# cmhungsteve/TA3N

Measured on NVIDIA H100. Metric: video-clips/sec fwd+bwd (B=256,T=5,D=2048), higher is better.
Workload: dtype tf32x3

## Files before the change

ta3n_b200/csrc/gemm_wgmma.cuh:

```cuda
#pragma once

#include <cuda.h>
#include <stdlib.h>

#include <algorithm>
#include <cmath>
#include <functional>
#include <map>
#include <tuple>

#include "seg_gemm.cuh"

namespace ta3n {

constexpr int TC_BM = 128, TC_BN = 128, TC_BK = 32;
constexpr int TC_THREADS = 384;
constexpr int TC_CONSUMER_WARPS = 8;
constexpr int TC_B_WARPS = 3;
constexpr int TC_B_THREADS = 32 * TC_B_WARPS;
constexpr int TC_PRODUCER_REGS = 40, TC_CONSUMER_REGS = 232;
static_assert(128 * TC_PRODUCER_REGS + 256 * TC_CONSUMER_REGS <= TC_THREADS * 168,
              "setmaxnreg budget exceeds the registers of one CTA");
constexpr int TC_XPOSE_PRODUCER_REGS = 64, TC_XPOSE_CONSUMER_REGS = 216;
static_assert(128 * TC_XPOSE_PRODUCER_REGS + 256 * TC_XPOSE_CONSUMER_REGS <= TC_THREADS * 168,
// ... 45 lines not shown
  } while (!done);
}
__device__ __forceinline__ void mbar_arrive(uint64_t* bar) {
  asm volatile("mbarrier.arrive.shared::cta.b64 _, [%0];" ::"r"(smem_u32(bar)) : "memory");
}
__device__ __forceinline__ void fence_barrier_init() { asm volatile("fence.mbarrier_init.release.cluster;" ::: "memory"); }
__device__ __forceinline__ void fence_proxy_async() { asm volatile("fence.proxy.async.shared::cta;" ::: "memory"); }

__device__ __forceinline__ void tma_load_2d(void* smem_dst, const CUtensorMap* map, uint64_t* bar, int c0, int c1) {
  asm volatile(
      "cp.async.bulk.tensor.2d.shared::cluster.global.mbarrier::complete_tx::bytes [%0], [%1, {%3, %4}], [%2];"
      ::"r"(smem_u32(smem_dst)), "l"(map), "r"(smem_u32(bar)), "r"(c0), "r"(c1)
      : "memory");
}
__device__ __forceinline__ void tma_load_3d(void* smem_dst, const CUtensorMap* map, uint64_t* bar, int c0, int c1,
                                            int c2) {
  asm volatile(
      "cp.async.bulk.tensor.3d.shared::cluster.global.mbarrier::complete_tx::bytes [%0], [%1, {%3, %4, %5}], [%2];"
      ::"r"(smem_u32(smem_dst)), "l"(map), "r"(smem_u32(bar)), "r"(c0), "r"(c1), "r"(c2)
      : "memory");
}
__device__ __forceinline__ void tma_prefetch_2d(const CUtensorMap* map, int c0, int c1) {
  asm volatile("cp.async.bulk.prefetch.tensor.2d.L2.global.tile [%0, {%1, %2}];" ::"l"(map), "r"(c0), "r"(c1) : "memory");
}
__device__ __forceinline__ void tma_prefetch_3d(const CUtensorMap* map, int c0, int c1, int c2) {
  asm volatile("cp.async.bulk.prefetch.tensor.3d.L2.global.tile [%0, {%1, %2, %3}];" ::"l"(map), "r"(c0), "r"(c1), "r"(c2)
               : "memory");
}
__device__ __forceinline__ void tma_prefetch_desc(const CUtensorMap* map) {
  asm volatile("prefetch.tensormap [%0];" ::"l"(map) : "memory");
}

__device__ __forceinline__ void sts4(uint32_t saddr, const float4 v) {
  asm volatile("st.shared.v4.f32 [%0], {%1, %2, %3, %4};" ::"r"(saddr), "f"(v.x), "f"(v.y), "f"(v.z), "f"(v.w) : "memory");
}
__device__ __forceinline__ float4 lds4(uint32_t saddr) {
  float4 v;
  asm volatile("ld.shared.v4.f32 {%0, %1, %2, %3}, [%4];" : "=f"(v.x), "=f"(v.y), "=f"(v.z), "=f"(v.w) : "r"(saddr) : "memory");
  return v;
}
__device__ __forceinline__ void wgmma_fence() { asm volatile("wgmma.fence.sync.aligned;" ::: "memory"); }
__device__ __forceinline__ void wgmma_commit() { asm volatile("wgmma.commit_group.sync.aligned;" ::: "memory"); }
template <int N>
__device__ __forceinline__ void wgmma_wait() {
  asm volatile("wgmma.wait_group.sync.aligned %0;" ::"n"(N) : "memory");
}

__device__ __forceinline__ uint64_t wgmma_desc(uint32_t tile_base, int kstep) {
  const uint32_t a = tile_base + (uint32_t)kstep * 32u;
  return (uint64_t)((a >> 4) & 0x3FFF) | ((uint64_t)1 << 16) | ((uint64_t)(1024 >> 4) << 32) | ((uint64_t)1 << 62);
}

__device__ __forceinline__ void wgmma_tf32(float (&d)[64], uint64_t adesc, uint64_t bdesc) {
  asm volatile(
      "{\n\t.reg .pred p;\n\t"
      "setp.ne.b32 p, %66, 0;\n\t"
      "wgmma.mma_async.sync.aligned.m64n128k8.f32.tf32.tf32 "
      "{%0, %1, %2, %3, %4, %5, %6, %7, %8, %9, %10, %11, %12, %13, %14, %15, %16, %17, %18, %19, %20, %21, %22, %23, %24, %25, %26, %27, %28, %29, %30, %31, %32, %33, %34, %35, %36, %37, %38, %39, %40, %41, %42, %43, %44, %45, %46, %47, %48, %49, %50, %51, %52, %53, %54, %55, %56, %57, %58, %59, %60, %61, %62, %63}, %64, %65, p, 1, 1;\n\t}"
      : "+f"(d[0]), "+f"(d[1]), "+f"(d[2]), "+f"(d[3]), "+f"(d[4]), "+f"(d[5]), "+f"(d[6]), "+f"(d[7]), "+f"(d[8]), "+f"(d[9]), "+f"(d[10]), "+f"(d[11]), "+f"(d[12]), "+f"(d[13]), "+f"(d[14]), "+f"(d[15]), "+f"(d[16]), "+f"(d[17]), "+f"(d[18]), "+f"(d[19]), "+f"(d[20]), "+f"(d[21]), "+f"(d[22]), "+f"(d[23]), "+f"(d[24]), "+f"(d[25]), "+f"(d[26]), "+f"(d[27]), "+f"(d[28]), "+f"(d[29]), "+f"(d[30]), "+f"(d[31]), "+f"(d[32]), "+f"(d[33]), "+f"(d[34]), "+f"(d[35]), "+f"(d[36]), "+f"(d[37]), "+f"(d[38]), "+f"(d[39]), "+f"(d[40]), "+f"(d[41]), "+f"(d[42]), "+f"(d[43]), "+f"(d[44]), "+f"(d[45]), "+f"(d[46]), "+f"(d[47]), "+f"(d[48]), "+f"(d[49]), "+f"(d[50]), "+f"(d[51]), "+f"(d[52]), "+f"(d[53]), "+f"(d[54]), "+f"(d[55]), "+f"(d[56]), "+f"(d[57]), "+f"(d[58]), "+f"(d[59]), "+f"(d[60]), "+f"(d[61]), "+f"(d[62]), "+f"(d[63])
      : "l"(adesc), "l"(bdesc), "r"(1)
      : "memory");
}
__device__ __forceinline__ void wgmma_tf32_rs(float (&d)[64], const uint32_t a0, const uint32_t a1, const uint32_t a2,
                                              const uint32_t a3, uint64_t bdesc) {
  asm volatile(
      "{\n\t.reg .pred p;\n\t"
      "setp.ne.b32 p, %69, 0;\n\t"
      "wgmma.mma_async.sync.aligned.m64n128k8.f32.tf32.tf32 "
      "{%0, %1, %2, %3, %4, %5, %6, %7, %8, %9, %10, %11, %12, %13, %14, %15, %16, %17, %18, %19, %20, %21, %22, %23, %24, %25, %26, %27, %28, %29, %30, %31, %32, %33, %34, %35, %36, %37, %38, %39, %40, %41, %42, %43, %44, %45, %46, %47, %48, %49, %50, %51, %52, %53, %54, %55, %56, %57, %58, %59, %60, %61, %62, %63}, {%64, %65, %66, %67}, %68, p, 1, 1;\n\t}"
      : "+f"(d[0]), "+f"(d[1]), "+f"(d[2]), "+f"(d[3]), "+f"(d[4]), "+f"(d[5]), "+f"(d[6]), "+f"(d[7]), "+f"(d[8]), "+f"(d[9]), "+f"(d[10]), "+f"(d[11]), "+f"(d[12]), "+f"(d[13]), "+f"(d[14]), "+f"(d[15]), "+f"(d[16]), "+f"(d[17]), "+f"(d[18]), "+f"(d[19]), "+f"(d[20]), "+f"(d[21]), "+f"(d[22]), "+f"(d[23]), "+f"(d[24]), "+f"(d[25]), "+f"(d[26]), "+f"(d[27]), "+f"(d[28]), "+f"(d[29]), "+f"(d[30]), "+f"(d[31]), "+f"(d[32]), "+f"(d[33]), "+f"(d[34]), "+f"(d[35]), "+f"(d[36]), "+f"(d[37]), "+f"(d[38]), "+f"(d[39]), "+f"(d[40]), "+f"(d[41]), "+f"(d[42]), "+f"(d[43]), "+f"(d[44]), "+f"(d[45]), "+f"(d[46]), "+f"(d[47]), "+f"(d[48]), "+f"(d[49]), "+f"(d[50]), "+f"(d[51]), "+f"(d[52]), "+f"(d[53]), "+f"(d[54]), "+f"(d[55]), "+f"(d[56]), "+f"(d[57]), "+f"(d[58]), "+f"(d[59]), "+f"(d[60]), "+f"(d[61]), "+f"(d[62]), "+f"(d[63])
      : "r"(a0), "r"(a1), "r"(a2), "r"(a3), "l"(bdesc), "r"(1)
      : "memory");
}
__device__ __forceinline__ void reg_fence(uint32_t& r) { asm volatile("" : "+r"(r)::"memory"); }
__device__ __forceinline__ float lds1(uint32_t saddr) {
  float v;
  asm volatile("ld.shared.f32 %0, [%1];" : "=f"(v) : "r"(saddr) : "memory");
  return v;
}
template <int N>
__device__ __forceinline__ void setmaxnreg_dec() { asm volatile("setmaxnreg.dec.sync.aligned.u32 %0;" ::"n"(N)); }
template <int N>
__device__ __forceinline__ void setmaxnreg_inc() { asm volatile("setmaxnreg.inc.sync.aligned.u32 %0;" ::"n"(N)); }

__device__ __forceinline__ uint32_t kmaj_chunk(int m, int kq) { return (uint32_t)(m * 128 + ((kq ^ (m & 7)) << 4)); }
__device__ __forceinline__ uint32_t mnmaj_chunk(int k, int mq) {
  return (uint32_t)((mq >> 3) * 4096 + k * 128 + (((mq & 7) ^ (k & 7)) << 4));
}
__device__ __forceinline__ float tf32_hi(float a) { return __uint_as_float(__float_as_uint(a) & 0xFFFFE000u); }
__device__ __forceinline__ float f4_at(const float4& v, int i) { return i == 0 ? v.x : i == 1 ? v.y : i == 2 ? v.z : v.w; }

__device__ __forceinline__ void tc_prep_blk(const int t, int* mq, int* kq) {
  *mq = (t & 3) | (((t >> 3) & 7) << 2);
  *kq = ((t >> 2) & 1) | ((((t >> 1) ^ (t >> 7)) & 1) << 1) | (((t >> 6) & 1) << 2);
}
__device__ __forceinline__ void tc_prep_load(const uint32_t base, const int t, float4 (&r)[4]) {
  int mq, kq;
  tc_prep_blk(t, &mq, &kq);
  const uint32_t p = base + (uint32_t)((mq >> 3) * 4096 + 512 * kq + (((mq & 7) ^ (4 * (kq & 1))) << 4));
#pragma unroll
  for (int i = 0; i < 4; ++i) r[i] = lds4((p ^ (i << 4)) + 128u * i);
}
__device__ __forceinline__ void tc_prep_store(const uint32_t base, const int t, const float4 (&r)[4]) {
  int mq, kq;
  tc_prep_blk(t, &mq, &kq);
  const uint32_t p = base + (uint32_t)(512 * mq + ((kq ^ (4 * (mq & 1))) << 4));
#pragma unroll
  for (int i = 0; i < 4; ++i)
    sts4((p ^ (i << 4)) + 128u * i, make_float4(f4_at(r[0], i), f4_at(r[1], i), f4_at(r[2], i), f4_at(r[3], i)));
}
static_assert(2 * TC_B_THREADS < 256 && 256 <= 3 * TC_B_THREADS, "tc_transpose_b moves two or three blocks per thread");
template <bool TWO_IN_FLIGHT>
__device__ __forceinline__ void tc_transpose_b(const uint32_t b_mn, const uint32_t b_k, const int t) {
  if (!TWO_IN_FLIGHT) {
#pragma unroll 1
    for (int blk = t; blk < 256; blk += TC_B_THREADS) {
      float4 r[4];
      tc_prep_load(b_mn, blk, r);
      tc_prep_store(b_k, blk, r);
    }
    return;
  }
  const bool third = t + 2 * TC_B_THREADS < 256;
  float4 r[4], q[4];
  tc_prep_load(b_mn, t, r);
  tc_prep_load(b_mn, t + TC_B_THREADS, q);
  tc_prep_store(b_k, t, r);
  if (third) tc_prep_load(b_mn, t + 2 * TC_B_THREADS, r);
  tc_prep_store(b_k, t + TC_B_THREADS, q);
  if (third) tc_prep_store(b_k, t + 2 * TC_B_THREADS, r);
}

template <bool A_KMAJ>
__device__ __forceinline__ uint32_t tc_a_thread_off(const int m, const int tq) {
  return A_KMAJ ? kmaj_chunk(m, 0) + 4u * tq : mnmaj_chunk(tq, m >> 2) + 4u * (m & 3);
}

template <bool A_KMAJ>
__device__ __forceinline__ void tc_load_a(const uint32_t a_base, const uint32_t off0, const uint32_t off1,
                                          uint32_t (&a)[16]) {
  const uint32_t p0 = a_base + off0, p1 = a_base + off1;
#pragma unroll
  for (int ks = 0; ks < TC_BK / 8; ++ks)
#pragma unroll
    for (int j = 0; j < 4; ++j) {
      const uint32_t row = j & 1, half = j >> 1;
      const uint32_t addr = A_KMAJ ? (p0 ^ ((2u * ks + half) << 4)) + 1024u * row
                                   : ((row ? p1 : p0) ^ (half << 6)) + 512u * half + 1024u * ks;
      a[4 * ks + j] = __float_as_uint(lds1(addr));
    }
}

#ifdef TA3N_TC_TIMELINE
constexpr int kTlCtas = 132, kTlSlabs = 64, kTlEvents = 9;
enum : int {
  TL_TMA_ISSUE,
  TL_FULL,
  TL_XPOSE_START,
  TL_XPOSE_END,
  TL_CONS_START,
  TL_READY,
  TL_RELEASED,
  TL_RETIRED,
  TL_FENCE,
};
__device__ unsigned long long g_tc_tl[kTlCtas][kTlSlabs][kTlEvents];
__device__ unsigned long long g_tc_tl_clk[kTlCtas][4];
__device__ __forceinline__ unsigned long long tl_globaltimer() {
  unsigned long long t;
  asm volatile("mov.u64 %0, %%globaltimer;" : "=l"(t));
  return t;
}
__device__ __forceinline__ void tl_stamp(const uint32_t slab, const int ev) {
  if (blockIdx.x < kTlCtas && slab < (uint32_t)kTlSlabs) g_tc_tl[blockIdx.x][slab][ev] = clock64();
}
__device__ __forceinline__ void tl_clock(const int at_end) {
  if (blockIdx.x < kTlCtas) {
    g_tc_tl_clk[blockIdx.x][2 * at_end] = tl_globaltimer();
    g_tc_tl_clk[blockIdx.x][2 * at_end + 1] = clock64();
  }
}
#define TA3N_TL(cond, slab, ev) \
  do {                          \
    if (cond) tl_stamp((uint32_t)(slab), (ev)); \
  } while (0)
#else
#define TA3N_TL(cond, slab, ev) ((void)0)
#endif

struct TcShared {
  uint64_t full_bar[kTcMaxStages];
  uint64_t empty_bar[kTcMaxStages];
};

template <int STAGES>
__device__ __forceinline__ void tc_pipe_init(TcShared* sh, const int readers = TC_CONSUMER_WARPS) {
  for (int s = 0; s < STAGES; ++s) {
    mbar_init(&sh->full_bar[s], 1);
    mbar_init(&sh->empty_bar[s], readers);
  }
  fence_barrier_init();
}

template <int STAGES, int STAGE_BYTES = TC_STAGE_BYTES>
__device__ __forceinline__ void tc_produce(const TileCtx& ctx, const CUtensorMap* __restrict__ maps, const bool a_kmaj,
                                           const bool b_kmaj, const int pad_flags, const int m0, const int n0,
                                           const int c_begin, const int n_iter, uint8_t* smem, TcShared* sh,
                                           const uint32_t slabs) {
  const Group& g = ctx.g;
  int seg = 0, k0 = 0;
  {
    int skip = c_begin;
    while (seg < g.seg_count) {
      const int nch = (ctx.seg[seg].len + TC_BK - 1) / TC_BK;
      if (skip < nch) {
        k0 = skip * TC_BK;
        break;
      }
      skip -= nch;
      ++seg;
    }
  }
  for (int it = 0; it < n_iter; ++it) {
    const uint32_t gl = slabs + (uint32_t)it;
    const int stage = (int)(gl % STAGES);
    const uint32_t phase = (gl / STAGES) & 1u;
    mbar_wait(&sh->empty_bar[stage], phase ^ 1u);
    TA3N_TL(true, gl, TL_TMA_ISSUE);
    mbar_expect_tx(&sh->full_bar[stage], TC_STAGE_BYTES);
    uint8_t* sA = smem + stage * STAGE_BYTES;
    uint8_t* sB = sA + TC_A_BYTES;
    const CUtensorMap* ma = &maps[ctx.seg[seg].amap];
    const CUtensorMap* mb = &maps[ctx.seg[seg].bmap];
    if (a_kmaj) {
      tma_load_2d(sA, ma, &sh->full_bar[stage], k0, m0);
    } else if (pad_flags & 1) {
      tma_load_3d(sA, ma, &sh->full_bar[stage], 0, k0, m0 >> 5);
    } else {
#pragma unroll
      for (int q = 0; q < TC_BM / 32; ++q) tma_load_2d(sA + q * 4096, ma, &sh->full_bar[stage], m0 + 32 * q, k0);
    }
    if (b_kmaj) {
      tma_load_2d(sB, mb, &sh->full_bar[stage], k0, n0);
    } else if (pad_flags & 2) {
      tma_load_3d(sB, mb, &sh->full_bar[stage], 0, k0, n0 >> 5);
    } else {
#pragma unroll
      for (int q = 0; q < TC_BN / 32; ++q) tma_load_2d(sB + q * 4096, mb, &sh->full_bar[stage], n0 + 32 * q, k0);
    }
    k0 += TC_BK;
    if (k0 >= ctx.seg[seg].len) {
      ++seg;
      k0 = 0;
    }
  }
}

__device__ __forceinline__ void tc_chunk_range(const TileCtx& ctx, int split, int* c_begin, int* n_iter) {
  const Group& g = ctx.g;
  int total_chunks = 0;
  for (int s = 0; s < g.seg_count; ++s) total_chunks += (ctx.seg[s].len + TC_BK - 1) / TC_BK;
  const int cps = (total_chunks + g.ksplit - 1) / g.ksplit;
  *c_begin = split * cps;
  *n_iter = max(0, min(total_chunks, *c_begin + cps) - *c_begin);
}

__device__ __forceinline__ void tc_decode(const TileCtx& ctx, const int tile, int* split, int* m0, int* n0) {
  const Group& g = ctx.g;
  int local = tile - g.tile_begin;
  const int per_split = g.tiles_m * g.tiles_n;
  *split = local / per_split;
  local -= *split * per_split;
  *m0 = (local / g.tiles_n) * TC_BM;
  *n0 = (local % g.tiles_n) * TC_BN;
}

__device__ __forceinline__ void frag_st2(float* p, const float x0, const float x1, const bool vec, const bool two) {
  if (vec) {
    *reinterpret_cast<float2*>(p) = make_float2(x0, x1);
  } else {
    p[0] = x0;
    if (two) p[1] = x1;
  }
}

template <int F>
__device__ __forceinline__ void frag_epilogue(const Group& g, const int m0, const int n0, const float (&v)[64]) {
  constexpr bool kFwd = F >= 0 && (F & ~(EPI_BIAS | EPI_RELU | EPI_DROP_RNG)) == 0;
  const int M = g.M, N = g.N, ldc = g.ldc;
  float* const C = g.C;
  const bool vec = (N % 2) == 0 && (ldc % 2) == 0 && (reinterpret_cast<uintptr_t>(C) & 7u) == 0;
  const float alpha = kFwd ? (g.alpha_dev ? g.alpha * __ldg(g.alpha_dev) : g.alpha) : 0.f;
  const float* const bias = g.bias;
  const uint64_t seed = g.seed, roff = g.rng_offset;
  const uint64_t step = (kFwd && (F & EPI_DROP_RNG) && g.step_dev) ? *g.step_dev : 0ull;
  const float dscale = g.drop_scale, dp = g.drop_p;
  const uint32_t thr = rng_threshold(dp);
  float b0[16], b1[16];
#pragma unroll
  for (int j = 0; j < 16; ++j) {
    const int n = n0 + 8 * j;
    b0[j] = kFwd && (F & EPI_BIAS) && n < N ? bias[n] : 0.f;
    b1[j] = kFwd && (F & EPI_BIAS) && n + 1 < N ? bias[n + 1] : 0.f;
  }
#pragma unroll
  for (int h = 0; h < 2; ++h) {
    const int m = m0 + 8 * h;
    if (m >= M) continue;
#pragma unroll
    for (int j = 0; j < 16; ++j) {
      const int n = n0 + 8 * j;
      if (n >= N) continue;
      const bool two = n + 1 < N;
      float x0 = v[4 * j + 2 * h], x1 = v[4 * j + 2 * h + 1];
      if (kFwd) {
        x0 *= alpha;
        x1 *= alpha;
        if (F & EPI_BIAS) {
          x0 += b0[j];
          x1 += b1[j];
        }
        if (F & EPI_RELU) {
          x0 = fmaxf(x0, 0.0f);
          x1 = fmaxf(x1, 0.0f);
        }
        if (F & EPI_DROP_RNG) {
          const uint64_t e = roff + (uint64_t)m * (uint64_t)N + (uint64_t)n;
          bool k0, k1;
          if ((e & 1ull) == 0) {
            const uint64_t hsh = rng_hash4(seed, step, e >> 2);
            k0 = rng_keep_bits(hsh, (int)(e & 3ull), thr);
            k1 = rng_keep_bits(hsh, (int)(e & 3ull) + 1, thr);
          } else {
            k0 = rng_keep(seed, step, e, dp);
            k1 = rng_keep(seed, step, e + 1, dp);
          }
          const float f0 = k0 ? dscale : 0.0f, f1 = k1 ? dscale : 0.0f;
          x0 = f0 != 0.0f ? x0 * f0 : 0.0f;
          x1 = f1 != 0.0f ? x1 * f1 : 0.0f;
        }
      } else {
        x0 = epilogue_t<F>(g, m, n, x0);
        if (two) x1 = epilogue_t<F>(g, m, n + 1, x1);
      }
      frag_st2(C + (size_t)m * ldc + n, x0, x1, vec, two);
    }
  }
}

__device__ __forceinline__ void frag_finish(const Group& g, const int split, const int tm0, const int tn0,
                                            const float (&v)[64]) {
  const int warp = threadIdx.x >> 5, lane = threadIdx.x & 31;
  const int m0 = tm0 + (warp >> 2) * 64 + (warp & 3) * 16 + (lane >> 2), n0 = tn0 + 2 * (lane & 3);
  if (g.ksplit > 1) {
    const int M = g.M, N = g.N;
    float* const part = g.partial + (size_t)split * M * N;
    const bool vec = (N % 2) == 0;
#pragma unroll
    for (int h = 0; h < 2; ++h)
#pragma unroll
      for (int j = 0; j < 16; ++j) {
        const int m = m0 + 8 * h, n = n0 + 8 * j;
        if (m < M && n < N) frag_st2(part + (size_t)m * N + n, v[4 * j + 2 * h], v[4 * j + 2 * h + 1], vec, n + 1 < N);
      }
    return;
  }
  TA3N_EPI_DISPATCH(g.flags, { frag_epilogue<EPI_F>(g, m0, n0, v); })
}


template <bool A_KMAJ, bool B_KMAJ>
__device__ __forceinline__ void tc_consume_slab(const uint32_t it, uint8_t* smem, TcShared* sh, uint64_t* kready_bar,
                                                uint64_t* kempty_bar, const uint32_t off0, const uint32_t off1,
                                                uint32_t (&a)[16], float (&d)[64], int& prev) {
  constexpr int kRaw = tc_raw_stages(B_KMAJ);
  const int stage = (int)(it % kRaw);
  const uint32_t parity = (it / kRaw) & 1u;
  const int kst = (int)(it % TC_KB_STAGES);
  TA3N_TL(threadIdx.x == 0, it, TL_CONS_START);
  mbar_wait(&sh->full_bar[stage], parity);
  if (!B_KMAJ) mbar_wait(&kready_bar[kst], (it / TC_KB_STAGES) & 1u);
  TA3N_TL(threadIdx.x == 0, it, TL_READY);
  const uint32_t a_base = smem_u32(smem + stage * TC_STAGE_BYTES);
  const uint32_t b_base = B_KMAJ ? a_base + TC_A_BYTES
                                 : smem_u32(smem + TC_RAW_STAGES * TC_STAGE_BYTES + kst * TC_B_BYTES);
  tc_load_a<A_KMAJ>(a_base, off0, off1, a);
#pragma unroll
  for (int j = 0; j < 16; ++j) reg_fence(a[j]);
  wgmma_fence();
#pragma unroll
  for (int ks = 0; ks < TC_BK / 8; ++ks) {
    const int f = 4 * ks;
    wgmma_tf32_rs(d, a[f], a[f + 1], a[f + 2], a[f + 3], wgmma_desc(b_base, ks));
  }
  wgmma_commit();
  if (!B_KMAJ) {
    __syncwarp();
    if ((threadIdx.x & 31) == 0) mbar_arrive(&sh->empty_bar[stage]);
    TA3N_TL(threadIdx.x == 0, it, TL_RELEASED);
  }
  wgmma_wait<1>();
  if (prev >= 0) {
    TA3N_TL(threadIdx.x == 0, it - 1, TL_RETIRED);
    __syncwarp();
    if ((threadIdx.x & 31) == 0) mbar_arrive(B_KMAJ ? &sh->empty_bar[prev] : &kempty_bar[prev]);
  }
  prev = B_KMAJ ? stage : kst;
}

template <bool A_KMAJ, bool B_KMAJ>
__global__ void __launch_bounds__(TC_THREADS, 1)
seg_gemm_tc_kernel(const __grid_constant__ GemmTable tab, const __grid_constant__ TcMaps maps,
                   const __grid_constant__ TcSegMaps segmaps, const int first_wave) {
  constexpr int kRaw = tc_raw_stages(B_KMAJ);
  extern __shared__ uint8_t tc_smem_raw[];
  __shared__ __align__(8) TcShared sh;
  __shared__ __align__(8) uint64_t kready_bar[TC_KB_STAGES];
  __shared__ __align__(8) uint64_t kempty_bar[TC_KB_STAGES];
  uint8_t* smem = reinterpret_cast<uint8_t*>((reinterpret_cast<uintptr_t>(tc_smem_raw) + 1023) & ~uintptr_t(1023));
  const int warp = threadIdx.x >> 5, lane = threadIdx.x & 31;
#ifdef TA3N_TC_TIMELINE
  if (threadIdx.x == 0) tl_clock(0);
#endif

  __shared__ TileCtx ctx;
  int tile = blockIdx.x;
  if (tile >= first_wave) tile = tab.total_tiles - 1 - (tile - first_wave);
  load_tile_ctx(tab, tile, &ctx, segmaps.a, segmaps.b);
  int split, m0, n0, c_begin, n_iter;
  tc_decode(ctx, tile, &split, &m0, &n0);
  tc_chunk_range(ctx, split, &c_begin, &n_iter);

  if (warp == TC_CONSUMER_WARPS && lane == 0) {
    for (int s = 0; s < TC_KB_STAGES; ++s) {
      mbar_init(&kready_bar[s], TC_B_WARPS);
      mbar_init(&kempty_bar[s], TC_CONSUMER_WARPS);
    }
    tc_pipe_init<kRaw>(&sh, TC_CONSUMER_WARPS + (B_KMAJ ? 0 : TC_B_WARPS));
  }
  __syncthreads();
  pdl_wait();

  if (warp >= TC_CONSUMER_WARPS) {
    setmaxnreg_dec<B_KMAJ ? TC_PRODUCER_REGS : TC_XPOSE_PRODUCER_REGS>();
    if (warp == TC_CONSUMER_WARPS) {
      if (lane == 0 && n_iter > 0)
        tc_produce<kRaw, TC_STAGE_BYTES>(ctx, maps.m, A_KMAJ, B_KMAJ, tab.pad_, m0, n0, c_begin, n_iter, smem, &sh, 0u);
    } else if (!B_KMAJ) {
      const int t = threadIdx.x - 32 * (TC_CONSUMER_WARPS + 1);
      const uint32_t kring = smem_u32(smem + TC_RAW_STAGES * TC_STAGE_BYTES);
      for (int it = 0; it < n_iter; ++it) {
        const int stage = it % TC_RAW_STAGES, kst = it % TC_KB_STAGES;
        mbar_wait(&sh.full_bar[stage], (uint32_t)(it / TC_RAW_STAGES) & 1u);
        TA3N_TL(t == 0, it, TL_FULL);
        mbar_wait(&kempty_bar[kst], ((uint32_t)(it / TC_KB_STAGES) & 1u) ^ 1u);
        TA3N_TL(t == 0, it, TL_XPOSE_START);
        tc_transpose_b<true>(smem_u32(smem + stage * TC_STAGE_BYTES) + TC_A_BYTES, kring + kst * TC_B_BYTES, t);
        TA3N_TL(t == 0, it, TL_FENCE);
        fence_proxy_async();
        __syncwarp();
        if (lane == 0) {
          mbar_arrive(&kready_bar[kst]);
          mbar_arrive(&sh.empty_bar[stage]);
        }
        TA3N_TL(t == 0, it, TL_XPOSE_END);
      }
    }
  } else {
    setmaxnreg_inc<B_KMAJ ? TC_CONSUMER_REGS : TC_XPOSE_CONSUMER_REGS>();
    const int r0 = (warp >> 2) * 64 + (warp & 3) * 16 + (lane >> 2);
    const uint32_t off0 = tc_a_thread_off<A_KMAJ>(r0, lane & 3), off1 = tc_a_thread_off<A_KMAJ>(r0 + 8, lane & 3);
    float d[64];
#pragma unroll
    for (int j = 0; j < 64; ++j) d[j] = 0.f;
    uint32_t a[2][16];
    int prev = -1;
    int it = 0;
    for (; it + 1 < n_iter; it += 2) {
      tc_consume_slab<A_KMAJ, B_KMAJ>((uint32_t)it, smem, &sh, kready_bar, kempty_bar, off0, off1, a[0], d, prev);
      tc_consume_slab<A_KMAJ, B_KMAJ>((uint32_t)(it + 1), smem, &sh, kready_bar, kempty_bar, off0, off1, a[1], d, prev);
    }
    if (it < n_iter)
      tc_consume_slab<A_KMAJ, B_KMAJ>((uint32_t)it, smem, &sh, kready_bar, kempty_bar, off0, off1, a[0], d, prev);
    wgmma_wait<0>();
    if (prev >= 0) {
      TA3N_TL(threadIdx.x == 0, n_iter - 1, TL_RETIRED);
      __syncwarp();
      if (lane == 0) mbar_arrive(B_KMAJ ? &sh.empty_bar[prev] : &kempty_bar[prev]);
    }
    frag_finish(ctx.g, split, m0, n0, d);
  }
#ifdef TA3N_TC_TIMELINE
  if (threadIdx.x == 0) tl_clock(1);
#endif
}

constexpr int X3_STAGES = 4;
constexpr int X3_STAGE_BYTES = TC_STAGE_BYTES + TC_B_BYTES;
constexpr int X3_CHUNK = 8;
static_assert(X3_CHUNK % 2 == 0, "the A fragment register sets alternate by slab within a chunk");
constexpr int x3_smem_bytes() { return X3_STAGES * X3_STAGE_BYTES + 1024; }

constexpr int kX3MaxCtas = 144;
constexpr int kX3MaxTasks = 1024;
struct X3Sched {
  int listed;
  unsigned short off[kX3MaxCtas + 1];
  unsigned short task[kX3MaxTasks];
};
static_assert(sizeof(GemmTable) + sizeof(TcMaps) + sizeof(TcSegMaps) + sizeof(X3Sched) + 256 <= 32764,
              "kernel parameters of the precise kernel exceed the 32 KB limit");

struct X3Slot {
  TileCtx ctx;
  int split, m0, n0, c_begin, n_iter;
};
constexpr int X3_SLOT_READERS = TC_CONSUMER_WARPS + 3;

__device__ __forceinline__ int x3_task(const X3Sched& sched, const int k) {
  return sched.listed ? (int)sched.task[sched.off[blockIdx.x] + k] : (int)(blockIdx.x + k * gridDim.x);
}

__device__ __forceinline__ void x3_stage(const GemmTable& tab, const TcSegMaps& sm, const int tile, X3Slot* sl) {
  const int lane = threadIdx.x & 31;
  int best = 0;
  for (int i = lane; i < tab.n_groups; i += 32)
    if (tile >= tab.g[i].tile_begin) best = max(best, i);
#pragma unroll
  for (int o = 16; o > 0; o >>= 1) best = max(best, __shfl_xor_sync(0xffffffffu, best, o));
  const int* src = reinterpret_cast<const int*>(&tab.g[best]);
  int* dst = reinterpret_cast<int*>(&sl->ctx.g);
  for (int i = lane; i < (int)(sizeof(Group) / sizeof(int)); i += 32) dst[i] = src[i];
  const int sb = tab.g[best].seg_begin, sc = tab.g[best].seg_count;
  for (int i = lane; i < sc; i += 32) {
    const Seg& s = tab.s[sb + i];
    SegLite l;
    l.A = s.A;
    l.B = s.B;
    l.len = s.len;
    l.lda = s.lda;
    l.ldb = s.ldb;
    l.amap = sm.a[sb + i];
    l.bmap = sm.b[sb + i];
    sl->ctx.seg[i] = l;
  }
  __syncwarp();
  if (lane == 0) {
    sl->ctx.gi = best;
    tc_decode(sl->ctx, tile, &sl->split, &sl->m0, &sl->n0);
    tc_chunk_range(sl->ctx, sl->split, &sl->c_begin, &sl->n_iter);
  }
  __syncwarp();
}

__device__ __forceinline__ void x3_split_sync() { asm volatile("bar.sync 2, 96;" ::: "memory"); }

template <bool B_KMAJ>
__device__ __forceinline__ void x3_split_b(const uint32_t b_raw, const uint32_t b_lo, const int t) {
  uint32_t src = b_raw;
  if (!B_KMAJ) {
    tc_transpose_b<false>(b_raw, b_lo, t);
    x3_split_sync();
    src = b_lo;
  }
#pragma unroll 2
  for (int c = t; c < TC_B_BYTES / 16; c += TC_B_THREADS) {
    const float4 v = lds4(src + 16u * c);
    if (!B_KMAJ) sts4(b_raw + 16u * c, v);
    sts4(b_lo + 16u * c, make_float4(v.x - tf32_hi(v.x), v.y - tf32_hi(v.y), v.z - tf32_hi(v.z), v.w - tf32_hi(v.w)));
  }
}

template <bool A_KMAJ>
__device__ __forceinline__ void x3_load_a(const uint32_t a_raw, const uint32_t off0, const uint32_t off1,
                                          uint32_t (&hi)[16], uint32_t (&lo)[16]) {
  uint32_t raw[16];
  tc_load_a<A_KMAJ>(a_raw, off0, off1, raw);
#pragma unroll
  for (int j = 0; j < 16; ++j) {
    const float a = __uint_as_float(raw[j]), h = tf32_hi(a);
    hi[j] = __float_as_uint(h);
    lo[j] = __float_as_uint(a - h);
  }
#pragma unroll
  for (int j = 0; j < 16; ++j) {
    reg_fence(hi[j]);
    reg_fence(lo[j]);
  }
}

template <bool A_KMAJ>
__device__ __forceinline__ void x3_consume_slab(const uint32_t gl, uint8_t* smem, TcShared* sh, uint64_t* ready_bar,
                                                const uint32_t off0, const uint32_t off1, uint32_t (&hi)[16],
                                                uint32_t (&lo)[16], float (&d)[64], int& prev) {
  const int stage = (int)(gl % X3_STAGES);
  const uint32_t parity = (gl / X3_STAGES) & 1u;
  mbar_wait(&sh->full_bar[stage], parity);
  mbar_wait(&ready_bar[stage], parity);
  const uint32_t a_raw = smem_u32(smem + stage * X3_STAGE_BYTES);
  const uint32_t b_hi = a_raw + TC_A_BYTES, b_lo = b_hi + TC_B_BYTES;
  x3_load_a<A_KMAJ>(a_raw, off0, off1, hi, lo);
  wgmma_fence();
#pragma unroll
  for (int ks = 0; ks < TC_BK / 8; ++ks) {
    const int f = 4 * ks;
    wgmma_tf32_rs(d, lo[f], lo[f + 1], lo[f + 2], lo[f + 3], wgmma_desc(b_hi, ks));
    wgmma_tf32_rs(d, hi[f], hi[f + 1], hi[f + 2], hi[f + 3], wgmma_desc(b_lo, ks));
    wgmma_tf32_rs(d, hi[f], hi[f + 1], hi[f + 2], hi[f + 3], wgmma_desc(b_hi, ks));
  }
  wgmma_commit();
  wgmma_wait<1>();
  if (prev >= 0) {
    __syncwarp();
    if ((threadIdx.x & 31) == 0) mbar_arrive(&sh->empty_bar[prev]);
  }
  prev = stage;
}

template <bool A_KMAJ, bool B_KMAJ>
__global__ void __launch_bounds__(TC_THREADS, 1)
seg_gemm_tc_x3_kernel(const __grid_constant__ GemmTable tab, const __grid_constant__ TcMaps maps,
                      const __grid_constant__ TcSegMaps segmaps, const __grid_constant__ X3Sched sched) {
  extern __shared__ uint8_t tc_smem_raw[];
  __shared__ __align__(8) TcShared sh;
  __shared__ __align__(8) uint64_t ready_bar[X3_STAGES];
  __shared__ __align__(8) uint64_t slot_full[2], slot_empty[2];
  __shared__ X3Slot slots[2];
  uint8_t* smem = reinterpret_cast<uint8_t*>((reinterpret_cast<uintptr_t>(tc_smem_raw) + 1023) & ~uintptr_t(1023));
  const int warp = threadIdx.x >> 5, lane = threadIdx.x & 31;
  const int n_tasks = sched.listed ? sched.off[blockIdx.x + 1] - sched.off[blockIdx.x]
                                   : (tab.total_tiles - (int)blockIdx.x + (int)gridDim.x - 1) / (int)gridDim.x;

  if (warp == TC_CONSUMER_WARPS) {
    if (lane == 0) {
      for (int s = 0; s < X3_STAGES; ++s) mbar_init(&ready_bar[s], TC_B_WARPS);
      for (int s = 0; s < 2; ++s) {
        mbar_init(&slot_full[s], 1);
        mbar_init(&slot_empty[s], X3_SLOT_READERS);
      }
      tc_pipe_init<X3_STAGES>(&sh);
    }
    __syncwarp();
    x3_stage(tab, segmaps, x3_task(sched, 0), &slots[0]);
    if (lane == 0) mbar_arrive(&slot_full[0]);
  }
  __syncthreads();
  pdl_wait();

  if (warp >= TC_CONSUMER_WARPS) {
    setmaxnreg_dec<TC_PRODUCER_REGS>();
    uint32_t slabs = 0;
    if (warp == TC_CONSUMER_WARPS) {
      for (int k = 0; k < n_tasks; ++k) {
        const int s = k & 1;
        if (k > 0) {
          mbar_wait(&slot_empty[s], ((uint32_t)(k >> 1) & 1u) ^ 1u);
          x3_stage(tab, segmaps, x3_task(sched, k), &slots[s]);
          if (lane == 0) mbar_arrive(&slot_full[s]);
        }
        const X3Slot& sl = slots[s];
        if (lane == 0 && sl.n_iter > 0)
          tc_produce<X3_STAGES, X3_STAGE_BYTES>(sl.ctx, maps.m, A_KMAJ, B_KMAJ, tab.pad_, sl.m0, sl.n0, sl.c_begin,
                                                sl.n_iter, smem, &sh, slabs);
        __syncwarp();
        slabs += (uint32_t)sl.n_iter;
      }
    } else {
      const int t = threadIdx.x - 32 * (TC_CONSUMER_WARPS + 1);
      for (int k = 0; k < n_tasks; ++k) {
        const int s = k & 1;
        mbar_wait(&slot_full[s], (uint32_t)(k >> 1) & 1u);
        const int n_iter = slots[s].n_iter;
        __syncwarp();
        if (lane == 0) mbar_arrive(&slot_empty[s]);
        for (int it = 0; it < n_iter; ++it) {
          const uint32_t gl = slabs + (uint32_t)it;
          const int stage = (int)(gl % X3_STAGES);
          mbar_wait(&sh.full_bar[stage], (gl / X3_STAGES) & 1u);
          const uint32_t b_raw = smem_u32(smem + stage * X3_STAGE_BYTES) + TC_A_BYTES;
          x3_split_b<B_KMAJ>(b_raw, b_raw + TC_B_BYTES, t);
          fence_proxy_async();
          __syncwarp();
          if (lane == 0) mbar_arrive(&ready_bar[stage]);
        }
        slabs += (uint32_t)n_iter;
      }
    }
  } else {
    setmaxnreg_inc<TC_CONSUMER_REGS>();
    const int r0 = (warp >> 2) * 64 + (warp & 3) * 16 + (lane >> 2);
    const uint32_t off0 = tc_a_thread_off<A_KMAJ>(r0, lane & 3), off1 = tc_a_thread_off<A_KMAJ>(r0 + 8, lane & 3);
    uint32_t slabs = 0;
    for (int k = 0; k < n_tasks; ++k) {
      const int s = k & 1;
      mbar_wait(&slot_full[s], (uint32_t)(k >> 1) & 1u);
      const int n_iter = slots[s].n_iter;
      float d[64], sum[64];
#pragma unroll
      for (int j = 0; j < 64; ++j) d[j] = sum[j] = 0.f;
      uint32_t hi[2][16], lo[2][16];
      int prev = -1;
      for (int c0 = 0; c0 < n_iter; c0 += X3_CHUNK) {
        const int c1 = min(n_iter, c0 + X3_CHUNK);
        for (int it = c0; it < c1; it += 2) {
          x3_consume_slab<A_KMAJ>(slabs + (uint32_t)it, smem, &sh, ready_bar, off0, off1, hi[0], lo[0], d, prev);
          if (it + 1 < c1)
            x3_consume_slab<A_KMAJ>(slabs + (uint32_t)(it + 1), smem, &sh, ready_bar, off0, off1, hi[1], lo[1], d, prev);
        }
        wgmma_wait<0>();
        __syncwarp();
        if (lane == 0) mbar_arrive(&sh.empty_bar[prev]);
        prev = -1;
#pragma unroll
        for (int j = 0; j < 64; ++j) {
          sum[j] += d[j];
          d[j] = 0.f;
        }
      }
      slabs += (uint32_t)n_iter;
      frag_finish(slots[s].ctx.g, slots[s].split, slots[s].m0, slots[s].n0, sum);
      __syncwarp();
      if (lane == 0) mbar_arrive(&slot_empty[s]);
    }
  }
}

typedef CUresult (*PFN_encodeTiled)(CUtensorMap*, CUtensorMapDataType, cuuint32_t, void*, const cuuint64_t*,
                                    const cuuint64_t*, const cuuint32_t*, const cuuint32_t*, CUtensorMapInterleave,
                                    CUtensorMapSwizzle, CUtensorMapL2promotion, CUtensorMapFloatOOBfill);

inline PFN_encodeTiled encode_fn() {
  static PFN_encodeTiled fn = []() -> PFN_encodeTiled {
    void* p = nullptr;
    cudaDriverEntryPointQueryResult q;
    if (cudaGetDriverEntryPoint("cuTensorMapEncodeTiled", &p, cudaEnableDefault, &q) != cudaSuccess) return nullptr;
    if (q != cudaDriverEntryPointSuccess) return nullptr;
    return reinterpret_cast<PFN_encodeTiled>(p);
  }();
  return fn;
}

struct DeviceInfo {
  int sm_count = 0;
  bool configured[4] = {false, false, false, false};
  bool x3_configured[4] = {false, false, false, false};
  bool eval_configured = false;
};
inline std::mutex& device_mu() {
  static std::mutex mu;
  return mu;
}
inline DeviceInfo* device_info() {
  static std::map<int, DeviceInfo> devs;
  int dev = 0;
  if (cudaGetDevice(&dev) != cudaSuccess) return nullptr;
  DeviceInfo& d = devs[dev];
  if (d.sm_count == 0) {
    if (cudaDeviceGetAttribute(&d.sm_count, cudaDevAttrMultiProcessorCount, dev) != cudaSuccess || d.sm_count <= 0)
      d.sm_count = 132;
  }
  return &d;
}
inline int device_sm_count() {
  std::lock_guard<std::mutex> lock(device_mu());
  DeviceInfo* d = device_info();
  return d ? d->sm_count : 132;
}

struct MapKey {
  const void* ptr;
  long inner, outer, ld;
  int box_inner, box_outer;
  int rank3;
  int raw;
  bool operator<(const MapKey& o) const {
    return std::tie(ptr, inner, outer, ld, box_inner, box_outer, rank3, raw) <
           std::tie(o.ptr, o.inner, o.outer, o.ld, o.box_inner, o.box_outer, o.rank3, o.raw);
  }
};

inline int encode_map(const MapKey& k, CUtensorMap* out) {
  static thread_local std::map<MapKey, CUtensorMap> cache;
  auto it = cache.find(k);
  if (it != cache.end()) {
    *out = it->second;
    return TA3N_OK;
  }
  PFN_encodeTiled fn = encode_fn();
  if (!fn) return fail(TA3N_ERR_CUDA, "cuTensorMapEncodeTiled entry point not available");
  static thread_local bool context_bound = false;
  if (!context_bound) {
    cudaFree(nullptr);
    context_bound = true;
  }
  cuuint64_t dims[3] = {(cuuint64_t)k.inner, (cuuint64_t)k.outer, 1};
  cuuint64_t strides[2] = {(cuuint64_t)k.ld * sizeof(float), 128};
  cuuint32_t box[3] = {(cuuint32_t)k.box_inner, (cuuint32_t)k.box_outer, 4};
  cuuint32_t estr[3] = {1, 1, 1};
  if (k.rank3) {
    dims[0] = 32;
    dims[2] = (cuuint64_t)(k.inner / 32);
  }
  CUresult r = fn(out, k.raw ? CU_TENSOR_MAP_DATA_TYPE_FLOAT32 : CU_TENSOR_MAP_DATA_TYPE_TFLOAT32, k.rank3 ? 3 : 2,
                  const_cast<void*>(k.ptr), dims, strides, box, estr,
                  CU_TENSOR_MAP_INTERLEAVE_NONE,
                  CU_TENSOR_MAP_SWIZZLE_128B,
                  CU_TENSOR_MAP_L2_PROMOTION_L2_256B,
                  CU_TENSOR_MAP_FLOAT_OOB_FILL_NONE);
  if (r != CUDA_SUCCESS) return fail(TA3N_ERR_CUDA, "cuTensorMapEncodeTiled failed with %d", (int)r);
  if (cache.size() > 4096) cache.clear();
  cache[k] = *out;
  return TA3N_OK;
}

inline bool tc_operand_ok(const float* p, int ld) {
  return p != nullptr && (reinterpret_cast<uintptr_t>(p) & 15u) == 0 && (ld % 4) == 0 && ld > 0;
}

inline void tc_seg_keys(const Seg& s, const Group& g, bool a_kmaj, bool b_kmaj, bool a3d, bool b3d, MapKey* ka,
                        MapKey* kb, bool raw = false) {
  const int rw = raw ? 1 : 0;
  *ka = a_kmaj ? MapKey{s.A, s.len, g.M, s.lda, TC_BK, TC_BM, 0, rw} : MapKey{s.A, g.M, s.len, s.lda, 32, TC_BK, a3d ? 1 : 0, rw};
  *kb = b_kmaj ? MapKey{s.B, s.len, g.N, s.ldb, TC_BK, TC_BN, 0, rw} : MapKey{s.B, g.N, s.len, s.ldb, 32, TC_BK, b3d ? 1 : 0, rw};
}

inline bool tc_group_ok(const GemmPlan& plan, const Group& g) {
  if (plan.load_flags != 0) return false;
  if ((long)g.M * g.N < 64L * 64L) return false;
  if (g.seg_count > kMaxSegs) return false;
  std::map<MapKey, int> maps;
  for (int i = 0; i < g.seg_count; ++i) {
    const Seg& s = plan.segs[g.seg_begin + i];
    if (!tc_operand_ok(s.A, s.lda) || !tc_operand_ok(s.B, s.ldb) || s.len <= 0) return false;
    MapKey ka, kb;
    tc_seg_keys(s, g, plan.a_kmaj, plan.b_kmaj, false, false, &ka, &kb);
    maps[ka] = maps[kb] = 0;
  }
  return (int)maps.size() <= kMaxMaps;
}

template <bool A_KMAJ, bool B_KMAJ>
inline int tc_launch_one(const GemmTable& tab, const TcMaps& maps, const TcSegMaps& sm, cudaStream_t stream,
                         const char* label) {
  constexpr int slot = (A_KMAJ ? 0 : 1) + (B_KMAJ ? 0 : 2);
  int first_wave = 132;
  {
    std::lock_guard<std::mutex> lock(device_mu());
    DeviceInfo* d = device_info();
    if (!d) return fail(TA3N_ERR_CUDA, "cudaGetDevice failed");
    if (!d->configured[slot]) {
      TA3N_CUDA(cudaFuncSetAttribute(seg_gemm_tc_kernel<A_KMAJ, B_KMAJ>, cudaFuncAttributeMaxDynamicSharedMemorySize,
                                     tc_smem_bytes(B_KMAJ)));
      d->configured[slot] = true;
    }
    first_wave = d->sm_count;
  }
  pre_launch(label, stream);
  launch_kernel(seg_gemm_tc_kernel<A_KMAJ, B_KMAJ>, tab.total_tiles, TC_THREADS, tc_smem_bytes(B_KMAJ), stream, tab,
                maps, sm, first_wave);
  return after_launch();
}

template <bool A_KMAJ, bool B_KMAJ>
inline int tc_launch_x3(const GemmTable& tab, const TcMaps& maps, const TcSegMaps& sm, const X3Sched& sched, int grid,
                        cudaStream_t stream, const char* label) {
  constexpr int slot = (A_KMAJ ? 0 : 1) + (B_KMAJ ? 0 : 2);
  {
    std::lock_guard<std::mutex> lock(device_mu());
    DeviceInfo* d = device_info();
    if (!d) return fail(TA3N_ERR_CUDA, "cudaGetDevice failed");
    if (!d->x3_configured[slot]) {
      TA3N_CUDA(cudaFuncSetAttribute(seg_gemm_tc_x3_kernel<A_KMAJ, B_KMAJ>, cudaFuncAttributeMaxDynamicSharedMemorySize,
                                     x3_smem_bytes()));
      d->x3_configured[slot] = true;
    }
  }
  pre_launch(label, stream);
// ... 298 lines not shown
```

Baseline: 1.284 million.

## Decouple A and B smem rings in tf32x3 kernel with early A release

Splits the shared single stage ring of the 3xTF32 wgmma kernel into separate A (3 stages) and B (5 stages, hi+lo) rings with their own full/ready/empty barriers. A stages are released as soon as consumers load A fragments into registers, while B stays held until its wgmma retires. This lets A and B run at different depths in the same smem budget. It also batches the B split loop loads ahead of stores, switches the transpose path variant, and picks different setmaxnreg budgets for the transposed B case. The extra barriers and a deeper B ring add sync overhead, and the new register split could cause consumer spills.

```diff
diff --git a/ta3n_b200/csrc/gemm_wgmma.cuh b/ta3n_b200/csrc/gemm_wgmma.cuh
--- a/ta3n_b200/csrc/gemm_wgmma.cuh
+++ b/ta3n_b200/csrc/gemm_wgmma.cuh
@@ -221,7 +221,7 @@
 }
 
 #ifdef TA3N_TC_TIMELINE
-constexpr int kTlCtas = 132, kTlSlabs = 64, kTlEvents = 9;
+constexpr int kTlCtas = 132, kTlSlabs = 64, kTlEvents = 11;
 enum : int {
   TL_TMA_ISSUE,
   TL_FULL,
@@ -233,6 +233,19 @@
   TL_RETIRED,
   TL_FENCE,
 };
+enum : int {
+  X3TL_TMA_B,
+  X3TL_TMA_A,
+  X3TL_FULL,
+  X3TL_XPOSED,
+  X3TL_SPLIT_END,
+  X3TL_READY,
+  X3TL_CONS_START,
+  X3TL_A_READY,
+  X3TL_B_READY,
+  X3TL_ISSUED,
+  X3TL_RETIRED,
+};
 __device__ unsigned long long g_tc_tl[kTlCtas][kTlSlabs][kTlEvents];
 __device__ unsigned long long g_tc_tl_clk[kTlCtas][4];
 __device__ __forceinline__ unsigned long long tl_globaltimer() {
@@ -271,25 +284,49 @@
   fence_barrier_init();
 }
 
+struct TcKCursor {
+  int seg, k0;
+};
+__device__ __forceinline__ TcKCursor tc_cursor(const TileCtx& ctx, int chunk) {
+  TcKCursor c{0, 0};
+  while (c.seg < ctx.g.seg_count) {
+    const int nch = (ctx.seg[c.seg].len + TC_BK - 1) / TC_BK;
+    if (chunk < nch) {
+      c.k0 = chunk * TC_BK;
+      break;
+    }
+    chunk -= nch;
+    ++c.seg;
+  }
+  return c;
+}
+__device__ __forceinline__ void tc_cursor_next(const TileCtx& ctx, TcKCursor& c) {
+  c.k0 += TC_BK;
+  if (c.k0 >= ctx.seg[c.seg].len) {
+    ++c.seg;
+    c.k0 = 0;
+  }
+}
+
+static_assert(TC_BM == TC_BN, "tc_tma_tile loads A and B tiles of the same row count");
+__device__ __forceinline__ void tc_tma_tile(uint8_t* dst, const CUtensorMap* map, uint64_t* bar, const bool kmaj,
+                                            const bool rank3, const int k0, const int row0) {
+  if (kmaj) {
+    tma_load_2d(dst, map, bar, k0, row0);
+  } else if (rank3) {
+    tma_load_3d(dst, map, bar, 0, k0, row0 >> 5);
+  } else {
+#pragma unroll
+    for (int q = 0; q < TC_BM / 32; ++q) tma_load_2d(dst + q * 4096, map, bar, row0 + 32 * q, k0);
+  }
+}
+
 template <int STAGES, int STAGE_BYTES = TC_STAGE_BYTES>
 __device__ __forceinline__ void tc_produce(const TileCtx& ctx, const CUtensorMap* __restrict__ maps, const bool a_kmaj,
                                            const bool b_kmaj, const int pad_flags, const int m0, const int n0,
                                            const int c_begin, const int n_iter, uint8_t* smem, TcShared* sh,
                                            const uint32_t slabs) {
-  const Group& g = ctx.g;
-  int seg = 0, k0 = 0;
-  {
-    int skip = c_begin;
-    while (seg < g.seg_count) {
-      const int nch = (ctx.seg[seg].len + TC_BK - 1) / TC_BK;
-      if (skip < nch) {
-        k0 = skip * TC_BK;
-        break;
-      }
-      skip -= nch;
-      ++seg;
-    }
-  }
+  TcKCursor cur = tc_cursor(ctx, c_begin);
   for (int it = 0; it < n_iter; ++it) {
     const uint32_t gl = slabs + (uint32_t)it;
     const int stage = (int)(gl % STAGES);
@@ -298,30 +335,10 @@
     TA3N_TL(true, gl, TL_TMA_ISSUE);
     mbar_expect_tx(&sh->full_bar[stage], TC_STAGE_BYTES);
     uint8_t* sA = smem + stage * STAGE_BYTES;
-    uint8_t* sB = sA + TC_A_BYTES;
-    const CUtensorMap* ma = &maps[ctx.seg[seg].amap];
-    const CUtensorMap* mb = &maps[ctx.seg[seg].bmap];
-    if (a_kmaj) {
-      tma_load_2d(sA, ma, &sh->full_bar[stage], k0, m0);
-    } else if (pad_flags & 1) {
-      tma_load_3d(sA, ma, &sh->full_bar[stage], 0, k0, m0 >> 5);
-    } else {
-#pragma unroll
-      for (int q = 0; q < TC_BM / 32; ++q) tma_load_2d(sA + q * 4096, ma, &sh->full_bar[stage], m0 + 32 * q, k0);
-    }
-    if (b_kmaj) {
-      tma_load_2d(sB, mb, &sh->full_bar[stage], k0, n0);
-    } else if (pad_flags & 2) {
-      tma_load_3d(sB, mb, &sh->full_bar[stage], 0, k0, n0 >> 5);
-    } else {
-#pragma unroll
-      for (int q = 0; q < TC_BN / 32; ++q) tma_load_2d(sB + q * 4096, mb, &sh->full_bar[stage], n0 + 32 * q, k0);
-    }
-    k0 += TC_BK;
-    if (k0 >= ctx.seg[seg].len) {
-      ++seg;
-      k0 = 0;
-    }
+    const SegLite& sg = ctx.seg[cur.seg];
+    tc_tma_tile(sA, &maps[sg.amap], &sh->full_bar[stage], a_kmaj, pad_flags & 1, cur.k0, m0);
+    tc_tma_tile(sA + TC_A_BYTES, &maps[sg.bmap], &sh->full_bar[stage], b_kmaj, pad_flags & 2, cur.k0, n0);
+    tc_cursor_next(ctx, cur);
   }
 }
 
@@ -564,11 +581,40 @@
 #endif
 }
 
-constexpr int X3_STAGES = 4;
-constexpr int X3_STAGE_BYTES = TC_STAGE_BYTES + TC_B_BYTES;
+constexpr int X3_A_STAGES = 3, X3_B_STAGES = 5;
+static_assert(X3_A_STAGES <= kTcMaxStages && X3_B_STAGES <= kTcMaxStages, "ring deeper than its barrier arrays");
+constexpr int X3_B_STAGE_BYTES = 2 * TC_B_BYTES;
 constexpr int X3_CHUNK = 8;
 static_assert(X3_CHUNK % 2 == 0, "the A fragment register sets alternate by slab within a chunk");
-constexpr int x3_smem_bytes() { return X3_STAGES * X3_STAGE_BYTES + 1024; }
+constexpr int x3_smem_bytes() { return X3_A_STAGES * TC_A_BYTES + X3_B_STAGES * X3_B_STAGE_BYTES + 1024; }
+struct X3Bars {
+  uint64_t a_full[X3_A_STAGES];
+  uint64_t a_empty[X3_A_STAGES];
+  uint64_t b_full[X3_B_STAGES];
+  uint64_t b_ready[X3_B_STAGES];
+  uint64_t b_empty[X3_B_STAGES];
+};
+
+__device__ __forceinline__ void x3_produce(const TileCtx& ctx, const CUtensorMap* __restrict__ maps, const bool a_kmaj,
+                                           const bool b_kmaj, const int pad_flags, const int m0, const int n0,
+                                           const int c_begin, const int n_iter, uint8_t* a_ring, uint8_t* b_ring,
+                                           X3Bars* bars, const uint32_t slabs) {
+  TcKCursor cur = tc_cursor(ctx, c_begin);
+  for (int it = 0; it < n_iter; ++it) {
+    const uint32_t gl = slabs + (uint32_t)it;
+    const int sa = (int)(gl % X3_A_STAGES), sb = (int)(gl % X3_B_STAGES);
+    const SegLite& sg = ctx.seg[cur.seg];
+    mbar_wait(&bars->b_empty[sb], ((gl / X3_B_STAGES) & 1u) ^ 1u);
+    TA3N_TL(true, gl, X3TL_TMA_B);
+    mbar_expect_tx(&bars->b_full[sb], TC_B_BYTES);
+    tc_tma_tile(b_ring + sb * X3_B_STAGE_BYTES, &maps[sg.bmap], &bars->b_full[sb], b_kmaj, pad_flags & 2, cur.k0, n0);
+    mbar_wait(&bars->a_empty[sa], ((gl / X3_A_STAGES) & 1u) ^ 1u);
+    TA3N_TL(true, gl, X3TL_TMA_A);
+    mbar_expect_tx(&bars->a_full[sa], TC_A_BYTES);
+    tc_tma_tile(a_ring + sa * TC_A_BYTES, &maps[sg.amap], &bars->a_full[sa], a_kmaj, pad_flags & 1, cur.k0, m0);
+    tc_cursor_next(ctx, cur);
+  }
+}
 
 constexpr int kX3MaxCtas = 144;
 constexpr int kX3MaxTasks = 1024;
@@ -624,20 +670,39 @@
 
 __device__ __forceinline__ void x3_split_sync() { asm volatile("bar.sync 2, 96;" ::: "memory"); }
 
+constexpr int X3_SPLIT_WORDS = TC_B_BYTES / 16;
+constexpr int X3_SPLIT_PER_THREAD = (X3_SPLIT_WORDS + TC_B_THREADS - 1) / TC_B_THREADS;
+constexpr int X3_SPLIT_BATCH = (X3_SPLIT_PER_THREAD + 1) / 2;
+static_assert(X3_SPLIT_WORDS % TC_B_THREADS != 0 &&
+              (X3_SPLIT_PER_THREAD - 1) * TC_B_THREADS < X3_SPLIT_WORDS, "only the last word of a thread is partial");
+template <bool B_KMAJ, int I0, int I1>
+__device__ __forceinline__ void x3_split_batch(const uint32_t src, const uint32_t b_raw, const uint32_t b_lo,
+                                               const int t) {
+  const bool last = (X3_SPLIT_PER_THREAD - 1) * TC_B_THREADS + t < X3_SPLIT_WORDS;
+  float4 v[I1 - I0];
+#pragma unroll
+  for (int i = I0; i < I1; ++i)
+    if (i < X3_SPLIT_PER_THREAD - 1 || last) v[i - I0] = lds4(src + 16u * (uint32_t)(t + TC_B_THREADS * i));
+#pragma unroll
+  for (int i = I0; i < I1; ++i) {
+    if (i == X3_SPLIT_PER_THREAD - 1 && !last) continue;
+    const uint32_t off = 16u * (uint32_t)(t + TC_B_THREADS * i);
+    const float4 w = v[i - I0];
+    if (!B_KMAJ) sts4(b_raw + off, w);
+    sts4(b_lo + off, make_float4(w.x - tf32_hi(w.x), w.y - tf32_hi(w.y), w.z - tf32_hi(w.z), w.w - tf32_hi(w.w)));
+  }
+}
 template <bool B_KMAJ>
-__device__ __forceinline__ void x3_split_b(const uint32_t b_raw, const uint32_t b_lo, const int t) {
+__device__ __forceinline__ void x3_split_b(const uint32_t b_raw, const uint32_t b_lo, const int t, const uint32_t gl) {
   uint32_t src = b_raw;
   if (!B_KMAJ) {
-    tc_transpose_b<false>(b_raw, b_lo, t);
+    tc_transpose_b<true>(b_raw, b_lo, t);
     x3_split_sync();
+    TA3N_TL(t == 0, gl, X3TL_XPOSED);
     src = b_lo;
   }
-#pragma unroll 2
-  for (int c = t; c < TC_B_BYTES / 16; c += TC_B_THREADS) {
-    const float4 v = lds4(src + 16u * c);
-    if (!B_KMAJ) sts4(b_raw + 16u * c, v);
-    sts4(b_lo + 16u * c, make_float4(v.x - tf32_hi(v.x), v.y - tf32_hi(v.y), v.z - tf32_hi(v.z), v.w - tf32_hi(v.w)));
-  }
+  x3_split_batch<B_KMAJ, 0, X3_SPLIT_BATCH>(src, b_raw, b_lo, t);
+  x3_split_batch<B_KMAJ, X3_SPLIT_BATCH, X3_SPLIT_PER_THREAD>(src, b_raw, b_lo, t);
 }
 
 template <bool A_KMAJ>
@@ -659,16 +724,22 @@
 }
 
 template <bool A_KMAJ>
-__device__ __forceinline__ void x3_consume_slab(const uint32_t gl, uint8_t* smem, TcShared* sh, uint64_t* ready_bar,
+__device__ __forceinline__ void x3_consume_slab(const uint32_t gl, uint8_t* a_ring, uint8_t* b_ring, X3Bars* bars,
                                                 const uint32_t off0, const uint32_t off1, uint32_t (&hi)[16],
                                                 uint32_t (&lo)[16], float (&d)[64], int& prev) {
-  const int stage = (int)(gl % X3_STAGES);
-  const uint32_t parity = (gl / X3_STAGES) & 1u;
-  mbar_wait(&sh->full_bar[stage], parity);
-  mbar_wait(&ready_bar[stage], parity);
-  const uint32_t a_raw = smem_u32(smem + stage * X3_STAGE_BYTES);
-  const uint32_t b_hi = a_raw + TC_A_BYTES, b_lo = b_hi + TC_B_BYTES;
+  const int sa = (int)(gl % X3_A_STAGES), sb = (int)(gl % X3_B_STAGES);
+  const uint32_t pb = (gl / X3_B_STAGES) & 1u;
+  TA3N_TL(threadIdx.x == 0, gl, X3TL_CONS_START);
+  mbar_wait(&bars->a_full[sa], (gl / X3_A_STAGES) & 1u);
+  TA3N_TL(threadIdx.x == 0, gl, X3TL_A_READY);
+  mbar_wait(&bars->b_ready[sb], pb);
+  mbar_wait(&bars->b_full[sb], pb);
+  TA3N_TL(threadIdx.x == 0, gl, X3TL_B_READY);
+  const uint32_t a_raw = smem_u32(a_ring + sa * TC_A_BYTES);
+  const uint32_t b_hi = smem_u32(b_ring + sb * X3_B_STAGE_BYTES), b_lo = b_hi + TC_B_BYTES;
   x3_load_a<A_KMAJ>(a_raw, off0, off1, hi, lo);
+  __syncwarp();
+  if ((threadIdx.x & 31) == 0) mbar_arrive(&bars->a_empty[sa]);
   wgmma_fence();
 #pragma unroll
   for (int ks = 0; ks < TC_BK / 8; ++ks) {
@@ -678,12 +749,14 @@
     wgmma_tf32_rs(d, hi[f], hi[f + 1], hi[f + 2], hi[f + 3], wgmma_desc(b_hi, ks));
   }
   wgmma_commit();
+  TA3N_TL(threadIdx.x == 0, gl, X3TL_ISSUED);
   wgmma_wait<1>();
   if (prev >= 0) {
+    TA3N_TL(threadIdx.x == 0, gl - 1, X3TL_RETIRED);
     __syncwarp();
-    if ((threadIdx.x & 31) == 0) mbar_arrive(&sh->empty_bar[prev]);
-  }
-  prev = stage;
+    if ((threadIdx.x & 31) == 0) mbar_arrive(&bars->b_empty[prev]);
+  }
+  prev = sb;
 }
 
 template <bool A_KMAJ, bool B_KMAJ>
@@ -691,23 +764,34 @@
 seg_gemm_tc_x3_kernel(const __grid_constant__ GemmTable tab, const __grid_constant__ TcMaps maps,
                       const __grid_constant__ TcSegMaps segmaps, const __grid_constant__ X3Sched sched) {
   extern __shared__ uint8_t tc_smem_raw[];
-  __shared__ __align__(8) TcShared sh;
-  __shared__ __align__(8) uint64_t ready_bar[X3_STAGES];
+  __shared__ __align__(8) X3Bars bars;
   __shared__ __align__(8) uint64_t slot_full[2], slot_empty[2];
   __shared__ X3Slot slots[2];
-  uint8_t* smem = reinterpret_cast<uint8_t*>((reinterpret_cast<uintptr_t>(tc_smem_raw) + 1023) & ~uintptr_t(1023));
+  uint8_t* a_ring = reinterpret_cast<uint8_t*>((reinterpret_cast<uintptr_t>(tc_smem_raw) + 1023) & ~uintptr_t(1023));
+  uint8_t* b_ring = a_ring + X3_A_STAGES * TC_A_BYTES;
   const int warp = threadIdx.x >> 5, lane = threadIdx.x & 31;
+#ifdef TA3N_TC_TIMELINE
+  if (threadIdx.x == 0) tl_clock(0);
+#endif
   const int n_tasks = sched.listed ? sched.off[blockIdx.x + 1] - sched.off[blockIdx.x]
                                    : (tab.total_tiles - (int)blockIdx.x + (int)gridDim.x - 1) / (int)gridDim.x;
 
   if (warp == TC_CONSUMER_WARPS) {
     if (lane == 0) {
-      for (int s = 0; s < X3_STAGES; ++s) mbar_init(&ready_bar[s], TC_B_WARPS);
+      for (int s = 0; s < X3_A_STAGES; ++s) {
+        mbar_init(&bars.a_full[s], 1);
+        mbar_init(&bars.a_empty[s], TC_CONSUMER_WARPS);
+      }
+      for (int s = 0; s < X3_B_STAGES; ++s) {
+        mbar_init(&bars.b_full[s], 1);
+        mbar_init(&bars.b_ready[s], TC_B_WARPS);
+        mbar_init(&bars.b_empty[s], TC_CONSUMER_WARPS);
+      }
       for (int s = 0; s < 2; ++s) {
         mbar_init(&slot_full[s], 1);
         mbar_init(&slot_empty[s], X3_SLOT_READERS);
       }
-      tc_pipe_init<X3_STAGES>(&sh);
+      fence_barrier_init();
     }
     __syncwarp();
     x3_stage(tab, segmaps, x3_task(sched, 0), &slots[0]);
@@ -717,7 +801,7 @@
   pdl_wait();
 
   if (warp >= TC_CONSUMER_WARPS) {
-    setmaxnreg_dec<TC_PRODUCER_REGS>();
+    setmaxnreg_dec<B_KMAJ ? TC_PRODUCER_REGS : TC_XPOSE_PRODUCER_REGS>();
     uint32_t slabs = 0;
     if (warp == TC_CONSUMER_WARPS) {
       for (int k = 0; k < n_tasks; ++k) {
@@ -729,8 +813,8 @@
         }
         const X3Slot& sl = slots[s];
         if (lane == 0 && sl.n_iter > 0)
-          tc_produce<X3_STAGES, X3_STAGE_BYTES>(sl.ctx, maps.m, A_KMAJ, B_KMAJ, tab.pad_, sl.m0, sl.n0, sl.c_begin,
-                                                sl.n_iter, smem, &sh, slabs);
+          x3_produce(sl.ctx, maps.m, A_KMAJ, B_KMAJ, tab.pad_, sl.m0, sl.n0, sl.c_begin, sl.n_iter, a_ring, b_ring,
+                     &bars, slabs);
         __syncwarp();
         slabs += (uint32_t)sl.n_iter;
       }
@@ -744,19 +828,22 @@
         if (lane == 0) mbar_arrive(&slot_empty[s]);
         for (int it = 0; it < n_iter; ++it) {
           const uint32_t gl = slabs + (uint32_t)it;
-          const int stage = (int)(gl % X3_STAGES);
-          mbar_wait(&sh.full_bar[stage], (gl / X3_STAGES) & 1u);
-          const uint32_t b_raw = smem_u32(smem + stage * X3_STAGE_BYTES) + TC_A_BYTES;
-          x3_split_b<B_KMAJ>(b_raw, b_raw + TC_B_BYTES, t);
+          const int sb = (int)(gl % X3_B_STAGES);
+          mbar_wait(&bars.b_full[sb], (gl / X3_B_STAGES) & 1u);
+          TA3N_TL(t == 0, gl, X3TL_FULL);
+          const uint32_t b_raw = smem_u32(b_ring + sb * X3_B_STAGE_BYTES);
+          x3_split_b<B_KMAJ>(b_raw, b_raw + TC_B_BYTES, t, gl);
+          TA3N_TL(t == 0, gl, X3TL_SPLIT_END);
           fence_proxy_async();
           __syncwarp();
-          if (lane == 0) mbar_arrive(&ready_bar[stage]);
+          if (lane == 0) mbar_arrive(&bars.b_ready[sb]);
+          TA3N_TL(t == 0, gl, X3TL_READY);
         }
         slabs += (uint32_t)n_iter;
       }
     }
   } else {
-    setmaxnreg_inc<TC_CONSUMER_REGS>();
+    setmaxnreg_inc<B_KMAJ ? TC_CONSUMER_REGS : TC_XPOSE_CONSUMER_REGS>();
     const int r0 = (warp >> 2) * 64 + (warp & 3) * 16 + (lane >> 2);
     const uint32_t off0 = tc_a_thread_off<A_KMAJ>(r0, lane & 3), off1 = tc_a_thread_off<A_KMAJ>(r0 + 8, lane & 3);
     uint32_t slabs = 0;
@@ -772,13 +859,15 @@
       for (int c0 = 0; c0 < n_iter; c0 += X3_CHUNK) {
         const int c1 = min(n_iter, c0 + X3_CHUNK);
         for (int it = c0; it < c1; it += 2) {
-          x3_consume_slab<A_KMAJ>(slabs + (uint32_t)it, smem, &sh, ready_bar, off0, off1, hi[0], lo[0], d, prev);
+          x3_consume_slab<A_KMAJ>(slabs + (uint32_t)it, a_ring, b_ring, &bars, off0, off1, hi[0], lo[0], d, prev);
           if (it + 1 < c1)
-            x3_consume_slab<A_KMAJ>(slabs + (uint32_t)(it + 1), smem, &sh, ready_bar, off0, off1, hi[1], lo[1], d, prev);
+            x3_consume_slab<A_KMAJ>(slabs + (uint32_t)(it + 1), a_ring, b_ring, &bars, off0, off1, hi[1], lo[1], d,
+                                    prev);
         }
         wgmma_wait<0>();
+        TA3N_TL(threadIdx.x == 0, slabs + (uint32_t)(c1 - 1), X3TL_RETIRED);
         __syncwarp();
-        if (lane == 0) mbar_arrive(&sh.empty_bar[prev]);
+        if (lane == 0) mbar_arrive(&bars.b_empty[prev]);
         prev = -1;
 #pragma unroll
         for (int j = 0; j < 64; ++j) {
@@ -792,6 +881,9 @@
       if (lane == 0) mbar_arrive(&slot_empty[s]);
     }
   }
+#ifdef TA3N_TC_TIMELINE
+  if (threadIdx.x == 0) tl_clock(1);
+#endif
 }
 
 typedef CUresult (*PFN_encodeTiled)(CUtensorMap*, CUtensorMapDataType, cuuint32_t, void*, const cuuint64_t*,
```

Result: no change. 1.285 million (median of 6 runs) (+0.1%).
